# sony/aki

Measured on AMD Instinct MI355X. Metric: image+text tokens/sec forward, AKI-4B, 336px img + 512 txt, higher is better.
Workload: dtype bf16

## Files before the change

aki_amd/_lib.py:

```python
from __future__ import annotations

import ctypes as C
import os
from typing import Optional

_HERE = os.path.dirname(os.path.abspath(__file__))
LIB_PATH = os.environ.get("AKI_MI355X_LIB") or os.path.join(_HERE, "lib", "libaki_mi355x.so")
LAB_LIB_PATH = os.path.join(_HERE, "lib", "libaki_mi355x_lab.so")

AKI_DT_BF16, AKI_DT_F32, AKI_DT_FP8_E4M3, AKI_DT_W8A16, AKI_DT_W4A16 = 0, 1, 2, 3, 4
AKI_ACT_NONE, AKI_ACT_GELU_ERF, AKI_ACT_GELU_TANH, AKI_ACT_SWIGLU = 0, 1, 2, 3
AKI_DEAD_ROWS_ZERO, AKI_DEAD_ROWS_UNIFORM = 0, 1
AKI_MAX_RECTS = 8
AKI_PLAN_STRIDE = 12
AKI_ABI_VERSION = 17
AKI_LOGITS_PROCESS_MAX_V = 131072


class AkiError(RuntimeError):
    pass


class MmaRect(C.Structure):
    _fields_ = [("row_lo", C.c_int32), ("row_hi", C.c_int32), ("col_lo", C.c_int32), ("col_hi", C.c_int32)]
# ... 108 lines not shown
                ("cache_len", C.c_void_p), ("col_valid_bits", C.c_void_p), ("workspace", C.c_void_p), ("workspace_bytes", C.c_size_t),
                ("n_layers", C.c_int32), ("nwords", C.c_int32), ("d", C.c_int32), ("H", C.c_int32), ("Dh", C.c_int32), ("F", C.c_int32),
                ("capacity", C.c_int32), ("max_keys", C.c_int32), ("scale", C.c_float), ("rms_eps", C.c_float), ("dtype", C.c_int32),
                ("batch", C.c_int32)]


SIGNATURES = {
    "aki_strerror": (C.c_char_p, [C.c_int]),
    "aki_abi_version": (C.c_int, []),
    "aki_mma_attn_core_workspace_bytes": (C.c_size_t, [C.c_int32] * 5),
    "aki_mma_attn_core_fwd": (C.c_int, [C.POINTER(MmaAttnCoreArgs), C.c_void_p, C.c_size_t, C.c_void_p]),
    "aki_mma_attn_workspace_bytes": (C.c_size_t, [C.c_int32] * 5),
    "aki_mma_attn_fwd": (C.c_int, [C.POINTER(MmaAttnArgs), C.c_void_p, C.c_size_t, C.c_void_p]),
    "aki_qkv_rope_fwd": (C.c_int, [C.POINTER(MmaAttnArgs), C.c_void_p, C.c_void_p, C.c_void_p, C.c_void_p, C.c_size_t, C.c_void_p]),
    "aki_attn_fwd": (C.c_int, [C.POINTER(AttnArgs), C.c_void_p, C.c_size_t, C.c_void_p]),
    "aki_linear_fwd": (C.c_int, [C.POINTER(LinearArgs), C.c_void_p]),
    "aki_linear_stats_workspace_bytes": (C.c_size_t, [C.c_int32, C.c_int32]),
    "aki_linear_splitk_workspace_bytes": (C.c_size_t, [C.c_int32, C.c_int32, C.c_int32]),
    "aki_linear_stats_counter_bytes": (C.c_size_t, [C.c_int32]),
    "aki_row_stats": (C.c_int, [C.c_void_p, C.c_int32, C.c_int32, C.c_int32, C.c_float, C.c_void_p, C.c_void_p, C.c_int32, C.c_void_p]),
    "aki_rmsnorm_fwd": (C.c_int, [C.c_void_p, C.c_void_p, C.c_void_p, C.c_int32, C.c_int32, C.c_int32, C.c_int32,
                                  C.c_float, C.c_int32, C.c_void_p]),
    "aki_layernorm_fwd": (C.c_int, [C.c_void_p, C.c_void_p, C.c_void_p, C.c_void_p, C.c_int32, C.c_int32, C.c_int32,
                                    C.c_int32, C.c_float, C.c_int32, C.c_void_p]),
    "aki_patch_embed_workspace_bytes": (C.c_size_t, [C.c_int32] * 4),
    "aki_patch_embed_fwd": (C.c_int, [C.c_void_p] * 5 + [C.c_int32] * 6 + [C.c_void_p, C.c_size_t, C.c_void_p]),
    "aki_connector_mlp_workspace_bytes": (C.c_size_t, [C.c_int32] * 4),
    "aki_connector_mlp_fwd": (C.c_int, [C.c_void_p] * 6 + [C.c_int32] * 3 + [C.c_float, C.c_int32, C.c_void_p, C.c_size_t,
                                                                            C.c_void_p]),
    "aki_connector_proj_fwd": (C.c_int, [C.c_void_p] * 6 + [C.c_int32] * 3 + [C.c_float, C.c_int32, C.c_void_p, C.c_size_t,
# ... 40 lines not shown
    "aki_quant_rows_fp8": (C.c_int, [C.c_void_p, C.c_void_p, C.c_float, C.c_void_p, C.c_void_p] + [C.c_int32] * 4 + [C.c_void_p]),
    "aki_quant_mxfp4": (C.c_int, [C.c_void_p, C.c_int32, C.c_int32, C.c_int32, C.c_void_p, C.c_void_p, C.c_void_p]),
    "aki_linear_w4_fwd": (C.c_int, [C.POINTER(LinearArgs), C.c_void_p, C.c_void_p, C.c_float, C.c_void_p]),
    "aki_splice_plan": (C.c_int, [C.c_void_p, C.c_int32, C.c_int32, C.c_int64, C.c_int64, C.c_int32, C.c_void_p, C.c_void_p]),
    "aki_splice_fwd": (C.c_int, [C.POINTER(SpliceArgs), C.c_void_p]),
    "aki_mma_mask_dense": (C.c_int, [C.c_void_p, C.c_int32, C.c_void_p, C.c_void_p, C.c_int32, C.c_int32, C.c_void_p,
                                     C.c_void_p]),
    "aki_greedy_pick": (C.c_int, [C.c_void_p, C.c_int32, C.c_int32, C.c_int64, C.c_void_p, C.c_int32, C.c_int64, C.c_void_p, C.c_void_p, C.c_void_p, C.c_int32,
                                  C.c_void_p, C.c_void_p, C.c_int32, C.c_void_p, C.c_void_p]),
    "aki_decoder_stack_workspace_bytes": (C.c_size_t, [C.c_int32] * 7),
    "aki_decoder_stack_fwd": (C.c_int, [C.POINTER(DecoderStackArgs), C.c_void_p]),
    "aki_siglip_stack_workspace_bytes": (C.c_size_t, [C.c_int32] * 4),
    "aki_siglip_stack_fwd": (C.c_int, [C.POINTER(SiglipStackArgs), C.c_void_p]),
    "aki_perceiver_stack_workspace_bytes": (C.c_size_t, [C.c_int32] * 6),
    "aki_perceiver_stack_fwd": (C.c_int, [C.POINTER(PerceiverStackArgs), C.c_void_p]),
    "aki_greedy_pick_embed": (C.c_int, [C.c_void_p, C.c_int32, C.c_int32, C.c_int64, C.c_void_p, C.c_int32, C.c_int64, C.c_void_p, C.c_void_p, C.c_void_p, C.c_int32,
                                        C.c_void_p, C.c_void_p, C.c_int32, C.c_void_p, C.c_void_p, C.c_void_p, C.c_int64, C.c_int64, C.c_int32, C.c_void_p,
                                        C.c_void_p]),
    "aki_logits_process": (C.c_int, [C.c_void_p, C.c_int32, C.c_int32, C.c_int32, C.c_int64, C.c_void_p, C.c_int64, C.c_void_p, C.c_int32,
                                     C.c_void_p, C.c_void_p, C.c_int32, C.c_void_p, C.c_float, C.c_int32, C.c_int32, C.c_void_p, C.c_int32,
                                     C.c_void_p, C.c_int32, C.c_void_p, C.c_int32, C.c_void_p, C.c_void_p, C.c_int32, C.c_int32, C.c_void_p]),
    "aki_greedy_pick_processed": (C.c_int, [C.c_void_p, C.c_int32, C.c_int32, C.c_int64, C.c_void_p, C.c_int32, C.c_int64, C.c_void_p, C.c_void_p,
                                            C.c_void_p, C.c_int32, C.c_void_p, C.c_void_p, C.c_int32, C.c_void_p, C.c_void_p, C.c_void_p, C.c_int64,
                                            C.c_int64, C.c_int32, C.c_void_p, C.c_void_p, C.c_int64, C.c_float, C.c_int32, C.c_int32, C.c_void_p,
                                            C.c_int32, C.c_void_p, C.c_int32, C.c_void_p, C.c_void_p, C.c_int32, C.c_int32, C.c_void_p]),
    "aki_sample_pick": (C.c_int, [C.c_void_p, C.c_int32, C.c_int32, C.c_int64, C.c_void_p, C.c_int32, C.c_int64, C.c_void_p, C.c_void_p,
                                  C.c_void_p, C.c_int32, C.c_void_p, C.c_void_p, C.c_int32, C.c_void_p, C.c_void_p, C.c_void_p, C.c_int64,
                                  C.c_int64, C.c_int32, C.c_void_p, C.c_void_p, C.c_int64, C.c_float, C.c_int32, C.c_int32, C.c_void_p,
                                  C.c_int32, C.c_void_p, C.c_int32, C.c_void_p, C.c_void_p, C.c_int32, C.c_int32, C.c_int32, C.c_float,
                                  C.c_int32, C.c_float, C.c_uint64, C.c_uint64, C.c_void_p, C.c_int64, C.c_void_p]),
# ... 144 lines not shown
```

aki_amd/csrc/api.hip:

```cpp
#include "aki_device.h"

namespace aki {
int linear_bf16(const aki_linear_args* a, hipStream_t stream);
size_t linear_stats_ws_bytes(int M, int n_out);
size_t linear_stats_cnt_bytes(int M);
int row_stats_launch(const void* x, int rows, int cols, int ldx, float eps, float* rstd, float* mean, hipStream_t s);
int linear_f32(const aki_linear_args* a, hipStream_t stream);
int qkv_rope_bf16(const aki_mma_attn_args* a, void* q, void* k, void* v, hipStream_t stream);
int qkv_rope_fp8(const aki_mma_attn_args* a, void* q, void* k, void* v, hipStream_t stream);
int linear_fp8(const aki_linear_args* a, hipStream_t stream);
int quant_rows_fp8_launch(const void* x, const void* rms_w, float eps, void* q, float* scale, int rows, int cols, int ldx, int ldq,
                          hipStream_t s);
int qkv_rope_f32(const aki_mma_attn_args* a, void* q, void* k, void* v, float* tmp, hipStream_t stream);
int attn_core_bf16(const aki_mma_attn_core_args* a, void* ws, size_t ws_bytes, hipStream_t stream);
int attn_core_f32(const aki_mma_attn_core_args* a, void* ws, size_t ws_bytes, hipStream_t stream, int causal);
int attn_nc_bf16(const aki_attn_args* a, hipStream_t stream);
int gemv_bf16(const aki_linear_args* a, const void* rms_w, float eps, hipStream_t stream);
int skinny_gemm_bf16(const aki_linear_args* a, const void* rms_w, float eps, hipStream_t stream);
int skinny_gemm_w8(const aki_linear_args* a, const void* rms_w, float eps, hipStream_t stream);
int quant_mxfp4_launch(const void* w, int N, int K, int ldw, uint8_t* wq, uint8_t* ws, hipStream_t s);
int gemv_w4(const aki_linear_args* a, const uint8_t* ws, const void* rms_w, float eps, hipStream_t stream);
int skinny_gemm_w4(const aki_linear_args* a, const uint8_t* ws, const void* rms_w, float eps, hipStream_t stream);
size_t decode_attn_ws_bytes(int B, int H, int Dh, int cap);
int decode_attn_split_launch(const void* q_or_qkv, const float* cos, const float* sin, const int* len, void* kc, void* vc, void* o,
                             const uint64_t* vbits, int nwords, int B, int H, int cap, int max_keys, float scale, bool fused,
                             void* ws, size_t ws_bytes, hipStream_t s);
int rope_append_launch(const void* qkv, const float* cos, const float* sin, const int* pos, const int* cache_len, void* q_out,
                       void* k_cache, void* v_cache, int B, int H, int Dh, int cap, int dtype, hipStream_t s);
int kv_cache_quant_fp8_launch(const void* src, int src_cap, void* dst, float* scale, int dst_cap, int slabs, int rows, hipStream_t s);
int decode_attn_split_fp8kv_launch(const void* qkv, const float* cos, const float* sin, const int* len, void* kc, void* vc, float* ks, float* vs,
                                   void* o, const uint64_t* vbits, int nwords, int B, int H, int cap, int max_keys, float scale, void* ws,
// ... 148 lines not shown
int aki_attn_fwd(const aki_attn_args* a, void* ws, size_t ws_bytes, void* stream) {
  AKI_CLEAR_ERR();
  AKI_CHECK_ARG(a && a->q && a->k && a->v && a->o);
  AKI_CHECK_ARG(a->B > 0 && a->H > 0 && a->Lq > 0 && a->Lk > 0 && a->Dh > 0 && a->scale > 0.f && dtype_ok(a->dtype));
  if (a->dtype == AKI_DT_BF16) return attn_nc_bf16(a, (hipStream_t)stream);
  const int64_t Dh = a->Dh;
  if (a->q_stride_t != Dh || a->k_stride_t != Dh || a->v_stride_t != Dh || a->q_stride_h != (int64_t)a->Lq * Dh ||
      a->k_stride_h != (int64_t)a->Lk * Dh || a->v_stride_h != (int64_t)a->Lk * Dh || a->Lq != a->Lk)
    return AKI_ERR_UNSUPPORTED;
  aki_mma_attn_core_args c = {};
  c.q = a->q; c.k = a->k; c.v = a->v; c.o = a->o; c.B = a->B; c.H = a->H; c.L = a->Lq; c.Dh = a->Dh; c.scale = a->scale;
  c.dtype = AKI_DT_F32; c.dead_rows = AKI_DEAD_ROWS_ZERO;
  return attn_core_f32(&c, ws, ws_bytes, (hipStream_t)stream, 0);
}

static size_t qkv_bytes(int B, int H, int L, int Dh, int dtype) {
  return aki_align_up((size_t)B * H * L * Dh * aki_elt_size(dtype), 256);
}

size_t aki_mma_attn_workspace_bytes(int32_t B, int32_t H, int32_t L, int32_t Dh, int32_t dtype) {
  size_t n = 3 * qkv_bytes(B, H, L, Dh, dtype) + aki_mma_attn_core_workspace_bytes(B, H, L, Dh, dtype);
  if (dtype == AKI_DT_F32) n += 3 * qkv_bytes(B, H, L, Dh, dtype);
  return n;
}

static int check_fused(const aki_mma_attn_args* a) {
  AKI_CHECK_ARG(a && a->x && a->w_qkv && a->cos && a->sin);
  AKI_CHECK_ARG(a->B > 0 && a->H > 0 && a->L > 0 && a->Dh > 0 && a->d_model > 0);
  AKI_CHECK_ARG(a->ldx >= a->d_model && a->ldw >= a->d_model && a->pos_rows > 0);
  AKI_CHECK_ARG(a->position_ids || a->pos_rows >= a->L);
// ... 643 lines not shown
```

aki_amd/csrc/attn_nc_bf16.hip:

```cpp
#include "aki_device.h"

namespace aki {

struct AttnNcParams {
  const bf16_t* q;
  const bf16_t* k;
  const bf16_t* v;
  bf16_t* o;
  long q_sb, q_sh, q_st;
  long k_sb, k_sh, k_st;
  long v_sb, v_sh, v_st;
  int B, H, Lq, Lk;
  int nqt;
  float scale_log2;
  float* lse;
};

__device__ __forceinline__ float max3_nc(float a, float b, float c) {
  float r;
  asm("v_max3_f32 %0, %1, %2, %3" : "=v"(r) : "v"(a), "v"(b), "v"(c));
  return r;
}

template <int NW, int DH>
__global__ __launch_bounds__(NW * 64, 2) void attn_nc_bf16_kernel(const AttnNcParams p) {
  constexpr int BQ = NW * 32, NT = NW * 64;
  constexpr int KS = (DH + 15) / 16;
  constexpr int DT = (DH + 31) / 32;
  constexpr int CPR = DH / 8;
  constexpr int KROW = DH == 96 ? 208 : (DH == 72 ? 176 : (DH == 64 ? 144 : 80));
  constexpr int VROW = 192;
  constexpr int KTILE = 64 * KROW, VTILE = 64 * VROW;
  constexpr int NCHUNK = 64 * CPR;
  constexpr int NCH = (NCHUNK + NT - 1) / NT;
  __shared__ __attribute__((aligned(16))) char smem[2 * KTILE + 2 * VTILE];
  char* const sK = smem;
  char* const sV = smem + 2 * KTILE;

  const int tid = threadIdx.x, lane = tid & 63;
// ... 9 lines not shown
    const u32x4 z = {0u, 0u, 0u, 0u};
    if (KS * 16 > DH)
      for (int r = tid; r < 2 * 64; r += NT) *(u32x4*)(sK + (r >> 6) * KTILE + (r & 63) * KROW + CPR * 16) = z;
    if (DT * 32 > DH) {
      constexpr int PADC = 12 - CPR;
      for (int e = tid; e < 2 * 64 * PADC; e += NT) {
        const int buf = e / (64 * PADC), rr = (e / PADC) & 63, pc = e % PADC;
        *(u32x4*)(sV + buf * VTILE + rr * VROW + (CPR + pc) * 16) = z;
      }
    }
  }

  const bf16_t* qrow = p.q + (size_t)b * p.q_sb + (size_t)head * p.q_sh + (size_t)min(row, Lq - 1) * p.q_st;
  const char* kb = (const char*)(p.k + (size_t)b * p.k_sb + (size_t)head * p.k_sh);
  const char* vb = (const char*)(p.v + (size_t)b * p.v_sb + (size_t)head * p.v_sh);

  bf16x8 qf[KS];
#pragma unroll
  for (int ks = 0; ks < KS; ++ks) {
    const int d = min(16 * ks + 8 * h, DH - 8);
    qf[ks] = *(const bf16x8*)(qrow + d);
  }

  f32x16 o[DT];
#pragma unroll
  for (int dt = 0; dt < DT; ++dt)
#pragma unroll
    for (int r = 0; r < 16; ++r) o[dt][r] = 0.f;
  float m_run = -1e30f, l_part = 0.f;

  constexpr int KCP = KROW / 16, VCP = VROW / 16;
  constexpr int KN = (64 * KCP + NT - 1) / NT, VN = (64 * VCP + NT - 1) / NT;
  auto issue_tile = [&](int j, int buf) {
    const int c0 = j * 64;
#pragma unroll
    for (int i = 0; i < KN; ++i) {
      const int c = i * NT + tid;
      const int kr = c / KCP, kc = c - kr * KCP;
      if (kc < CPR && c < 64 * KCP) {
        const size_t trow = (size_t)min(c0 + kr, Lk - 1);
        __builtin_amdgcn_global_load_lds(AKI_GLOBAL_PTR(kb + trow * p.k_st * 2 + kc * 16), AKI_LDS_PTR(sK + buf * KTILE + (i * NT + wave * 64) * 16), 16, 0, 0);
      }
    }
#pragma unroll
    for (int i = 0; i < VN; ++i) {
      const int c = i * NT + tid;
      const int kr = c / VCP, kc = c - kr * VCP;
      if (kc < CPR && c < 64 * VCP) {
        const size_t trow = (size_t)min(c0 + kr, Lk - 1);
        __builtin_amdgcn_global_load_lds(AKI_GLOBAL_PTR(vb + trow * p.v_st * 2 + kc * 16), AKI_LDS_PTR(sV + buf * VTILE + (i * NT + wave * 64) * 16), 16, 0, 0);
      }
    }
  };

  const int koff = l31 * KROW + h * 16;
  const int voff = (4 * h + ((lane & 15) >> 2)) * VROW + (16 * ((lane >> 4) & 1) + 4 * (lane & 3)) * 2;
  const int jend = (Lk + 63) >> 6;

  __syncthreads();
  issue_tile(0, 0);
  __builtin_amdgcn_s_waitcnt(0x0F70);
  __syncthreads();

  for (int j = 0; j < jend; ++j) {
    if (j + 1 < jend) issue_tile(j + 1, (j + 1) & 1);
// ... 98 lines not shown
    bf16_t* orow = p.o + ((size_t)(b * Lq + row) * p.H + head) * DH + 4 * h;
#pragma unroll
    for (int dt = 0; dt < DT; ++dt)
#pragma unroll
      for (int q4 = 0; q4 < 4; ++q4) {
        const int d = dt * 32 + q4 * 8 + 4 * h;
        if (d < DH) {
          u32x2 pk = {pack_bf16x2(o[dt][4 * q4] * inv, o[dt][4 * q4 + 1] * inv), pack_bf16x2(o[dt][4 * q4 + 2] * inv, o[dt][4 * q4 + 3] * inv)};
          *(u32x2*)(orow + dt * 32 + q4 * 8) = pk;
        }
      }
    if (p.lse && h == 0) p.lse[(size_t)bh * Lq + row] = (m_run + __builtin_amdgcn_logf(l_tot)) * 0.69314718055994530942f;
  }
}

int attn_nc_bf16(const aki_attn_args* a, hipStream_t stream) {
  AttnNcParams p = {(const bf16_t*)a->q, (const bf16_t*)a->k, (const bf16_t*)a->v, (bf16_t*)a->o,
                    a->q_stride_b, a->q_stride_h, a->q_stride_t, a->k_stride_b, a->k_stride_h, a->k_stride_t,
                    a->v_stride_b, a->v_stride_h, a->v_stride_t, a->B, a->H, a->Lq, a->Lk, 0,
                    a->scale * 1.44269504088896340736f, a->lse};
  constexpr int NW = 4;
  p.nqt = (a->Lq + NW * 32 - 1) / (NW * 32);
  const long ss[] = {a->q_stride_b, a->q_stride_h, a->q_stride_t, a->k_stride_b, a->k_stride_h, a->k_stride_t,
                     a->v_stride_b, a->v_stride_h, a->v_stride_t};
  for (long s : ss)
    if (s % 8) return AKI_ERR_ALIGNMENT;
  AKI_CHECK_ALIGN16(a->q); AKI_CHECK_ALIGN16(a->k); AKI_CHECK_ALIGN16(a->v);
  if ((uintptr_t)a->o & 7) return AKI_ERR_ALIGNMENT;
  const dim3 grid(a->B * a->H * p.nqt), block(NW * 64);
  AKI_CLEAR_ERR();
  switch (a->Dh) {
    case 96: hipLaunchKernelGGL((attn_nc_bf16_kernel<NW, 96>), grid, block, 0, stream, p); break;
    case 72: hipLaunchKernelGGL((attn_nc_bf16_kernel<NW, 72>), grid, block, 0, stream, p); break;
    case 64: hipLaunchKernelGGL((attn_nc_bf16_kernel<NW, 64>), grid, block, 0, stream, p); break;
    case 32: hipLaunchKernelGGL((attn_nc_bf16_kernel<NW, 32>), grid, block, 0, stream, p); break;
    default: return AKI_ERR_UNSUPPORTED;
  }
  AKI_LAUNCH_CHECK();
  return AKI_OK;
}

}
```

aki_amd/csrc/stack.hip:

```cpp
#include <hip/hip_runtime.h>

#include "aki_device.h"

namespace {

inline char* carve(char*& p, size_t bytes) {
  char* r = p;
  p += aki_align_up(bytes, 256);
  return r;
}

}

extern "C" {

size_t aki_decoder_stack_workspace_bytes(int32_t B, int32_t H, int32_t L, int32_t Dh, int32_t d, int32_t F, int32_t keep_kv) {
  if (B <= 0 || H <= 0 || L <= 0 || Dh <= 0 || d <= 0 || F <= 0) return 0;
  const size_t M = (size_t)B * L, head = aki_align_up(M * H * Dh * 2, 256);
  return head * (keep_kv ? 1 : 3)
         + aki_align_up(M * (size_t)H * Dh * 2, 256)
         + 2 * aki_align_up(M * (size_t)d * 2, 256)
         + aki_align_up(M * (size_t)F * 2, 256)
         + 3 * aki_align_up(M * 4, 256)
         + aki_mma_attn_core_workspace_bytes(B, H, L, Dh, AKI_DT_BF16);
// ... 205 lines not shown
    rc = aki_attn_fwd(&at, attn_ws, attn_ws_bytes, stream);
    if (rc) return rc;
    aki_linear_args oa = {};
    oa.x = ao; oa.w = ly.w_out; oa.residual = cur; oa.y = lat[0]; oa.M = n2; oa.N = D; oa.K = inner; oa.ldx = inner; oa.ldw = inner; oa.ldy = D; oa.ldr = D;
    oa.act = AKI_ACT_NONE; oa.dtype = AKI_DT_BF16;
    rc = aki_linear_fwd(&oa, stream);
    if (rc) return rc;
    rc = aki_connector_mlp_fwd(lat[0], ly.ff_ln_w, ly.ff_ln_b, ly.ff_w1, ly.ff_w2, lat[1], n2, D, a->d_ff, a->eps, AKI_DT_BF16, mlp_ws, mlp_ws_bytes, stream);
    if (rc) return rc;
    cur = lat[1];
  }
  if (a->proj_w) return aki_connector_proj_fwd(cur, a->norm_w, a->norm_b, a->proj_w, a->proj_b, a->out, n2, D, a->D_out, a->eps, AKI_DT_BF16, mlp_ws, mlp_ws_bytes, stream);
  return aki_layernorm_fwd(cur, a->norm_w, a->norm_b, a->out, n2, D, D, D, a->eps, AKI_DT_BF16, stream);
}

}
```

aki_amd/helpers.py:

```python
from __future__ import annotations

from dataclasses import dataclass
from typing import Optional

import torch
import torch.nn.functional as F
from torch import nn

from . import ops
from . import train_ops as TR

try:
    from transformers.modeling_outputs import CausalLMOutputWithPast
except Exception:
    @dataclass
    class CausalLMOutputWithPast:
        loss: Optional[torch.Tensor] = None
        logits: Optional[torch.Tensor] = None
        past_key_values: Optional[object] = None
        hidden_states: Optional[object] = None
        attentions: Optional[object] = None

        def __getitem__(self, i):
            return [v for v in (self.loss, self.logits, self.past_key_values) if v is not None][i]
# ... 82 lines not shown
            self.layers.append(nn.ModuleList([PerceiverAttention(dim=dim, dim_head=dim_head, heads=heads),
                                              FeedForward(dim=dim, mult=ff_mult)]))
        self.norm = nn.LayerNorm(dim)

    use_layer_stack = True

    def _can_stack(self, x) -> bool:
        if not (self.use_layer_stack and ops.stack_enabled() and x.is_cuda and x.dtype == torch.bfloat16 and x.is_contiguous()):
            return False
        eps = self.norm.eps
        for attn, ff in self.layers:
            if (attn.norm_media.eps != eps or attn.norm_latents.eps != eps or ff[0].eps != eps
                    or attn.heads != self.layers[0][0].heads or attn.dim_head != self.layers[0][0].dim_head):
                return False
        return not ops.python_must_run_between(self.layers)

    def _forward_stack(self, x, latents):
        tb = getattr(self, "_stack_table", None)
        if tb is None:
            tb = self._stack_table = ops.LayerTable(ops.L.PerceiverLayer)
        live = []
        for attn, ff in self.layers:
            live += [attn.norm_media.weight, attn.norm_media.bias, attn.norm_latents.weight, attn.norm_latents.bias, attn.to_q.weight,
                     attn.to_kv.weight, attn.to_out.weight, ff[0].weight, ff[0].bias, ff[1].weight, ff[3].weight]
        sig = (tuple(map(id, live)), ops.params_signature(live))
        if tb.sig != sig:
            rows = []
            for attn, ff in self.layers:
                rows.append((attn.norm_media.weight, attn.norm_media.bias, attn.norm_latents.weight, attn.norm_latents.bias, attn.to_q.weight,
                             attn.to_kv.weight, attn.to_out.weight, ff[0].weight, ff[0].bias, ff[1].weight, ff[3].weight))
            for r in rows:
                for t_ in r:
                    if t_ is not None and not t_.is_contiguous():
                        raise ops.AkiError("perceiver stack: weights must be contiguous")
            tb.get(rows)
            tb.sig = sig
        a0 = self.layers[0][0]
        proj = self.projection
        return ops.perceiver_stack(tb.arr, len(self.layers), x.reshape(-1, x.shape[-1]), latents.reshape(-1, latents.shape[-1]), self.norm.weight, self.norm.bias,
                                   None if proj is None else proj.weight, None if proj is None else proj.bias, a0.heads, a0.dim_head,
                                   self.layers[0][1][1].weight.shape[0], a0.scale, self.norm.eps)

    def forward(self, x):
        b, T, Fr, v = x.shape[:4]
        if exists(self.frame_embs):
            x = x + self.frame_embs[:Fr][None, None, :, None, :]
        x = x.reshape(b, T, Fr * v, x.shape[-1])
        if exists(self.media_time_embs):
            x = x + self.media_time_embs[:T]
        latents = self.latents.to(x.dtype)[None, None].expand(b, T, -1, -1).contiguous()
        if _ag(latents, *self.parameters()):
            for attn, ff in self.layers:
                latents = attn(x, latents)
                hmid = TR.GeluFn.apply(TR.linear(TR.layernorm(latents, ff[0].weight, ff[0].bias, ff[0].eps), ff[1].weight))
                latents = TR.linear(hmid, ff[3].weight, None, latents)
            latents = TR.layernorm(latents, self.norm.weight, self.norm.bias, self.norm.eps)
            if exists(self.projection):
                return TR.linear(latents, self.projection.weight, self.projection.bias, None)
            return latents
        if b * T == 1 and self._can_stack(x):
            return self._forward_stack(x, latents).view(b, T, latents.shape[2], -1)
        for attn, ff in self.layers:
            latents = attn(x, latents)
            latents = ops.connector_mlp(latents, ff[0].weight, ff[0].bias, ff[1].weight, ff[3].weight, ff[0].eps)
        if exists(self.projection):
            return ops.connector_proj(latents, self.norm.weight, self.norm.bias, self.projection.weight,
                                      self.projection.bias, self.norm.eps)
        return ops.layernorm(latents, self.norm.weight, self.norm.bias, self.norm.eps)


def _table_dims(given: Optional[torch.Tensor], declared_rows, declared_cols, what: str):
    if given is None:
        if declared_rows is None or declared_cols is None:
            raise AssertionError(f"{what}: without a ready-made tensor both sizes have to be given")
        return int(declared_rows), int(declared_cols)
    rows, cols = given.shape
    for declared, actual in ((declared_rows, rows), (declared_cols, cols)):
        if declared is not None and declared != actual:
            raise AssertionError(f"{what}: the tensor is {rows} x {cols}, which contradicts the declared size {declared}")
# ... 102 lines not shown
```

aki_amd/ops.py:

```python
from __future__ import annotations

import ctypes as C
import threading
from dataclasses import dataclass
from typing import Optional, Tuple

import torch

from . import _lib as L
from ._lib import AkiError

ACT_NONE, ACT_GELU_ERF, ACT_GELU_TANH, ACT_SWIGLU = L.AKI_ACT_NONE, L.AKI_ACT_GELU_ERF, L.AKI_ACT_GELU_TANH, L.AKI_ACT_SWIGLU
DEAD_ROWS_ZERO, DEAD_ROWS_UNIFORM = L.AKI_DEAD_ROWS_ZERO, L.AKI_DEAD_ROWS_UNIFORM


def _dt(t: torch.Tensor) -> int:
    if t.dtype == torch.bfloat16:
        return L.AKI_DT_BF16
    if t.dtype == torch.float32:
        return L.AKI_DT_F32
    raise AkiError(f"unsupported dtype {t.dtype}: the AKI HIP path computes in bf16 or f32")


def _dev(*ts: Optional[torch.Tensor]) -> torch.device:
# ... 254 lines not shown
    q, k, v = q.contiguous(), k.contiguous(), v.contiguous()
    o = torch.empty((B, Lq, H * Dh), dtype=q.dtype, device=dev)
    lse = torch.empty((B, H, Lq), dtype=torch.float32, device=dev) if return_lse else None
    lib = L.load()
    ws = _ws(lib.aki_mma_attn_core_workspace_bytes(B, H, Lq, Dh, _dt(q)), dev)
    a = L.MmaAttnCoreArgs(_ptr(q), _ptr(k), _ptr(v), _ptr(o), _ptr(lse), _ptr(table.rects), _ptr(table.col_valid_bits),
                          _ptr(table.seq_lens), table.max_rects, B, H, Lq, Dh, float(scale), _dt(q), dead_rows,
                          0 if cap == Lq else cap)
    end = _TAP.begin(("mma_attn_core", B, H, Lq, Dh)) if (_TAP is not None and _TAP.want(("mma_attn_core",))) else None
    L.check(lib.aki_mma_attn_core_fwd(C.byref(a), _ptr(ws), ws.numel(), _stream()), "aki_mma_attn_core_fwd")
    if end is not None:
        end.record()
    return (o, lse) if return_lse else o


def attention(q: torch.Tensor, k: torch.Tensor, v: torch.Tensor, scale: float, return_lse: bool = False):
    dev = _dev(q, k, v)
    B, Lq, H, Dh = q.shape
    Lk = k.shape[1]
    o = torch.empty((B, Lq, H * Dh), dtype=q.dtype, device=dev)
    lib = L.load()
    if q.dtype == torch.float32:
        if Lq != Lk:
            qp = torch.zeros((B, Lk, H, Dh), dtype=q.dtype, device=dev)
            qp[:, :Lq] = q
            return attention(qp, k, v, scale)[:, :Lq].contiguous()
        q, k, v = (t_.permute(0, 2, 1, 3).contiguous() for t_ in (q, k, v))
        st = lambda t_: (t_.stride(0), t_.stride(1), t_.stride(2))
    else:
        for t_ in (q, k, v):
            if t_.stride(3) != 1:
                raise AkiError("attention: channel stride must be 1")
        st = lambda t_: (t_.stride(0), t_.stride(2), t_.stride(1))
    ws = _ws(B * H * Dh * 4 + 256, dev)
# ... 648 lines not shown
    if x.dtype != torch.bfloat16 or not x.is_contiguous() or not latents.is_contiguous() or x.dim() != 2 or latents.dim() != 2:
        raise AkiError("perceiver_stack: contiguous bf16 [n, D] tensors")
    lib = L.load()
    n1, D = x.shape
    n2 = latents.shape[0]
    D_out = D if proj_w is None else proj_w.shape[0]
    out = torch.empty((n2, D_out), dtype=x.dtype, device=dev)
    ws = _scratch(int(lib.aki_perceiver_stack_workspace_bytes(n1, n2, D, heads, dim_head, d_ff)), dev)
    off = (-ws.data_ptr()) % 256
    a = L.PerceiverStackArgs(table_arr, n_layers, _ptr(x), _ptr(latents), _ptr(norm_w), _ptr(norm_b), _ptr(proj_w), _ptr(proj_b), _ptr(out), n1, n2, D, heads,
                             dim_head, d_ff, D_out, float(scale), float(eps), ws.data_ptr() + off, ws.numel() - off)
    L.check(lib.aki_perceiver_stack_fwd(C.byref(a), _stream()), "aki_perceiver_stack_fwd")
    return out


def quant_rows_fp8(x: torch.Tensor, rms_weight: Optional[torch.Tensor] = None, eps: float = 0.0):
    dev = _dev(x, rms_weight)
    if x.dtype != torch.bfloat16:
        raise AkiError("quant_rows_fp8 takes bf16 input")
    x2 = _rows2d(x)
    rows, cols = x2.shape
    q = torch.empty((rows, cols), dtype=torch.uint8, device=dev)
    s = torch.empty((rows,), dtype=torch.float32, device=dev)
    L.check(L.load().aki_quant_rows_fp8(_ptr(x2), _ptr(rms_weight), float(eps), _ptr(q), _ptr(s), rows, cols, x2.stride(0),
                                        q.stride(0), _stream()), "aki_quant_rows_fp8")
    return q, s


def linear_fp8(xq: torch.Tensor, xs: torch.Tensor, wq: torch.Tensor, ws: torch.Tensor, bias: Optional[torch.Tensor] = None,
               residual: Optional[torch.Tensor] = None, act: int = ACT_NONE, out_shape=None) -> torch.Tensor:
# ... 307 lines not shown
```

include/aki_mi355x.h:

```cpp
#ifndef AKI_MI355X_H
#define AKI_MI355X_H

#include <stddef.h>
#include <stdint.h>

#ifdef __cplusplus
extern "C" {
#endif

#define AKI_ABI_VERSION 17

typedef enum {
  AKI_OK = 0,
  AKI_ERR_INVALID_ARG = -1,
  AKI_ERR_UNSUPPORTED = -2,
  AKI_ERR_ALIGNMENT = -3,
  AKI_ERR_WORKSPACE = -4,
  AKI_ERR_LAUNCH = -5
} aki_status;

typedef enum {
  AKI_DT_BF16 = 0,
  AKI_DT_F32 = 1,
  AKI_DT_FP8_E4M3 = 2,
// ... 73 lines not shown
typedef struct {
  const void* q;
  const void* k;
  const void* v;
  void* o;
  int64_t q_stride_b, q_stride_h, q_stride_t;
  int64_t k_stride_b, k_stride_h, k_stride_t;
  int64_t v_stride_b, v_stride_h, v_stride_t;
  int32_t B, H, Lq, Lk, Dh;
  float scale;
  int32_t dtype;
  float* lse;
} aki_attn_args;

int aki_attn_fwd(const aki_attn_args* args, void* workspace, size_t workspace_bytes, void* stream);

typedef struct {
  const void* x;
  const void* w;
  const void* bias;
  const void* residual;
  void* y;
  int32_t M, N, K;
  int32_t ldx, ldw, ldy, ldr;
  int32_t res_row_mod;
  int32_t act;
  int32_t dtype;
  const float* x_scale;
  const float* w_scale;
  const void* w2;
// ... 306 lines not shown
  const void* norm_w;
  const void* norm_b;
  const void* proj_w;
  const void* proj_b;
  void* out;
  int32_t n1, n2, D, heads, dim_head, d_ff, D_out;
  float scale;
  float eps;
  void* workspace;
  size_t workspace_bytes;
} aki_perceiver_stack_args;

size_t aki_perceiver_stack_workspace_bytes(int32_t n1, int32_t n2, int32_t D, int32_t heads, int32_t dim_head, int32_t d_ff);
int aki_perceiver_stack_fwd(const aki_perceiver_stack_args* args, void* stream);

int aki_greedy_pick_embed(const void* logits, int32_t B, int32_t V, int64_t ld, const int64_t* eos_ids, int32_t n_eos, int64_t pad_token_id,
                          uint8_t* done, int64_t* next_ids, int64_t* tokens, int32_t tokens_ld, int32_t* cache_len, const int32_t* start_len,
                          int32_t advance, int32_t* done_at, const void* embed_weight, const void* additional_weight, int64_t max_original_id,
                          int64_t num_additional, int32_t d, void* next_embeds, void* stream);

#define AKI_LOGITS_PROCESS_MAX_V 131072
int aki_logits_process(const void* logits, int32_t dtype, int32_t B, int32_t V, int64_t ld, float* out, int64_t ld_out, const int64_t* tokens,
                       int32_t tokens_ld, const int32_t* cache_len, const int32_t* start_len, int32_t step, const uint8_t* done,
                       float repetition_penalty, int32_t no_repeat_ngram_size, int32_t min_length, const int64_t* eos_ids, int32_t n_eos,
                       const int64_t* suppress_ids, int32_t n_suppress, const int64_t* begin_suppress_ids, int32_t n_begin_suppress,
                       const int64_t* bad_ids, const int32_t* bad_offsets, int32_t n_bad, int32_t n_bad_ids, void* stream);

int aki_greedy_pick_processed(const void* logits, int32_t B, int32_t V, int64_t ld, const int64_t* eos_ids, int32_t n_eos, int64_t pad_token_id,
                              uint8_t* done, int64_t* next_ids, int64_t* tokens, int32_t tokens_ld, int32_t* cache_len, const int32_t* start_len,
                              int32_t advance, int32_t* done_at, const void* embed_weight, const void* additional_weight, int64_t max_original_id,
// ... 19 lines not shown
```

Before: 131,000.

## Split perceiver attention into media and latent KV segments to avoid concat

Adds a two-segment key/value attention kernel so the perceiver resampler can attend over media keys and latent keys without materializing the concatenated KV tensor. The latent K/V projection is merged with the Q projection into one stacked GEMM per layer. Optionally, all layers' media KV projections can be folded into one GEMM with the layernorm applied as row scale and shift. The cost is a per-load branch in the kernel, cached stacked weight copies, and a path limited to head dim 64.

```diff
diff --git a/aki_amd/_lib.py b/aki_amd/_lib.py
--- a/aki_amd/_lib.py
+++ b/aki_amd/_lib.py
@@ -146,6 +146,7 @@
     "aki_mma_attn_fwd": (C.c_int, [C.POINTER(MmaAttnArgs), C.c_void_p, C.c_size_t, C.c_void_p]),
     "aki_qkv_rope_fwd": (C.c_int, [C.POINTER(MmaAttnArgs), C.c_void_p, C.c_void_p, C.c_void_p, C.c_void_p, C.c_size_t, C.c_void_p]),
     "aki_attn_fwd": (C.c_int, [C.POINTER(AttnArgs), C.c_void_p, C.c_size_t, C.c_void_p]),
+    "aki_attn_kv2_fwd": (C.c_int, [C.POINTER(AttnArgs), C.c_void_p, C.c_void_p] + [C.c_int64] * 6 + [C.c_int32, C.c_void_p]),
     "aki_linear_fwd": (C.c_int, [C.POINTER(LinearArgs), C.c_void_p]),
     "aki_linear_stats_workspace_bytes": (C.c_size_t, [C.c_int32, C.c_int32]),
     "aki_linear_splitk_workspace_bytes": (C.c_size_t, [C.c_int32, C.c_int32, C.c_int32]),
@@ -216,6 +217,8 @@
     "aki_siglip_stack_fwd": (C.c_int, [C.POINTER(SiglipStackArgs), C.c_void_p]),
     "aki_perceiver_stack_workspace_bytes": (C.c_size_t, [C.c_int32] * 6),
     "aki_perceiver_stack_fwd": (C.c_int, [C.POINTER(PerceiverStackArgs), C.c_void_p]),
+    "aki_perceiver_stack_shared_workspace_bytes": (C.c_size_t, [C.c_int32] * 7),
+    "aki_perceiver_stack_shared_fwd": (C.c_int, [C.POINTER(PerceiverStackArgs)] + [C.c_void_p] * 5),
     "aki_greedy_pick_embed": (C.c_int, [C.c_void_p, C.c_int32, C.c_int32, C.c_int64, C.c_void_p, C.c_int32, C.c_int64, C.c_void_p, C.c_void_p, C.c_void_p, C.c_int32,
                                         C.c_void_p, C.c_void_p, C.c_int32, C.c_void_p, C.c_void_p, C.c_void_p, C.c_int64, C.c_int64, C.c_int32, C.c_void_p,
                                         C.c_void_p]),
diff --git a/aki_amd/csrc/api.hip b/aki_amd/csrc/api.hip
--- a/aki_amd/csrc/api.hip
+++ b/aki_amd/csrc/api.hip
@@ -15,6 +15,7 @@
 int attn_core_bf16(const aki_mma_attn_core_args* a, void* ws, size_t ws_bytes, hipStream_t stream);
 int attn_core_f32(const aki_mma_attn_core_args* a, void* ws, size_t ws_bytes, hipStream_t stream, int causal);
 int attn_nc_bf16(const aki_attn_args* a, hipStream_t stream);
+int attn_nc_bf16_kv2(const aki_attn_args* a, const void* k2, const void* v2, const int64_t* s2, int Lk1, hipStream_t stream);
 int gemv_bf16(const aki_linear_args* a, const void* rms_w, float eps, hipStream_t stream);
 int skinny_gemm_bf16(const aki_linear_args* a, const void* rms_w, float eps, hipStream_t stream);
 int skinny_gemm_w8(const aki_linear_args* a, const void* rms_w, float eps, hipStream_t stream);
@@ -193,6 +194,16 @@
   return attn_core_f32(&c, ws, ws_bytes, (hipStream_t)stream, 0);
 }
 
+int aki_attn_kv2_fwd(const aki_attn_args* a, const void* k2, const void* v2, int64_t k2_stride_b, int64_t k2_stride_h, int64_t k2_stride_t,
+                     int64_t v2_stride_b, int64_t v2_stride_h, int64_t v2_stride_t, int32_t Lk1, void* stream) {
+  AKI_CLEAR_ERR();
+  AKI_CHECK_ARG(a && a->q && a->k && a->v && a->o && k2 && v2);
+  AKI_CHECK_ARG(a->B > 0 && a->H > 0 && a->Lq > 0 && a->Dh > 0 && a->scale > 0.f && Lk1 > 0 && Lk1 < a->Lk);
+  if (a->dtype != AKI_DT_BF16) return AKI_ERR_UNSUPPORTED;
+  const int64_t s2[6] = {k2_stride_b, k2_stride_h, k2_stride_t, v2_stride_b, v2_stride_h, v2_stride_t};
+  return attn_nc_bf16_kv2(a, k2, v2, s2, Lk1, (hipStream_t)stream);
+}
+
 static size_t qkv_bytes(int B, int H, int L, int Dh, int dtype) {
   return aki_align_up((size_t)B * H * L * Dh * aki_elt_size(dtype), 256);
 }
diff --git a/aki_amd/csrc/attn_nc_bf16.hip b/aki_amd/csrc/attn_nc_bf16.hip
--- a/aki_amd/csrc/attn_nc_bf16.hip
+++ b/aki_amd/csrc/attn_nc_bf16.hip
@@ -14,6 +14,11 @@
   int nqt;
   float scale_log2;
   float* lse;
+  const bf16_t* k2;
+  const bf16_t* v2;
+  long k2_sb, k2_sh, k2_st;
+  long v2_sb, v2_sh, v2_st;
+  int Lk1;
 };
 
 __device__ __forceinline__ float max3_nc(float a, float b, float c) {
@@ -22,7 +27,7 @@
   return r;
 }
 
-template <int NW, int DH>
+template <int NW, int DH, bool SEG2 = false>
 __global__ __launch_bounds__(NW * 64, 2) void attn_nc_bf16_kernel(const AttnNcParams p) {
   constexpr int BQ = NW * 32, NT = NW * 64;
   constexpr int KS = (DH + 15) / 16;
@@ -62,6 +67,8 @@
   const bf16_t* qrow = p.q + (size_t)b * p.q_sb + (size_t)head * p.q_sh + (size_t)min(row, Lq - 1) * p.q_st;
   const char* kb = (const char*)(p.k + (size_t)b * p.k_sb + (size_t)head * p.k_sh);
   const char* vb = (const char*)(p.v + (size_t)b * p.v_sb + (size_t)head * p.v_sh);
+  const char* kb2 = SEG2 ? (const char*)(p.k2 + (size_t)b * p.k2_sb + (size_t)head * p.k2_sh) : nullptr;
+  const char* vb2 = SEG2 ? (const char*)(p.v2 + (size_t)b * p.v2_sb + (size_t)head * p.v2_sh) : nullptr;
 
   bf16x8 qf[KS];
 #pragma unroll
@@ -86,8 +93,10 @@
       const int c = i * NT + tid;
       const int kr = c / KCP, kc = c - kr * KCP;
       if (kc < CPR && c < 64 * KCP) {
-        const size_t trow = (size_t)min(c0 + kr, Lk - 1);
-        __builtin_amdgcn_global_load_lds(AKI_GLOBAL_PTR(kb + trow * p.k_st * 2 + kc * 16), AKI_LDS_PTR(sK + buf * KTILE + (i * NT + wave * 64) * 16), 16, 0, 0);
+        const int trow = min(c0 + kr, Lk - 1);
+        const char* src = kb + (size_t)trow * p.k_st * 2;
+        if (SEG2 && trow >= p.Lk1) src = kb2 + (size_t)(trow - p.Lk1) * p.k2_st * 2;
+        __builtin_amdgcn_global_load_lds(AKI_GLOBAL_PTR(src + kc * 16), AKI_LDS_PTR(sK + buf * KTILE + (i * NT + wave * 64) * 16), 16, 0, 0);
       }
     }
 #pragma unroll
@@ -95,8 +104,10 @@
       const int c = i * NT + tid;
       const int kr = c / VCP, kc = c - kr * VCP;
       if (kc < CPR && c < 64 * VCP) {
-        const size_t trow = (size_t)min(c0 + kr, Lk - 1);
-        __builtin_amdgcn_global_load_lds(AKI_GLOBAL_PTR(vb + trow * p.v_st * 2 + kc * 16), AKI_LDS_PTR(sV + buf * VTILE + (i * NT + wave * 64) * 16), 16, 0, 0);
+        const int trow = min(c0 + kr, Lk - 1);
+        const char* src = vb + (size_t)trow * p.v_st * 2;
+        if (SEG2 && trow >= p.Lk1) src = vb2 + (size_t)(trow - p.Lk1) * p.v2_st * 2;
+        __builtin_amdgcn_global_load_lds(AKI_GLOBAL_PTR(src + kc * 16), AKI_LDS_PTR(sV + buf * VTILE + (i * NT + wave * 64) * 16), 16, 0, 0);
       }
     }
   };
@@ -225,7 +236,7 @@
   }
 }
 
-int attn_nc_bf16(const aki_attn_args* a, hipStream_t stream) {
+static int attn_nc_launch(const aki_attn_args* a, const void* k2, const void* v2, const int64_t* s2, int Lk1, hipStream_t stream) {
   AttnNcParams p = {(const bf16_t*)a->q, (const bf16_t*)a->k, (const bf16_t*)a->v, (bf16_t*)a->o,
                     a->q_stride_b, a->q_stride_h, a->q_stride_t, a->k_stride_b, a->k_stride_h, a->k_stride_t,
                     a->v_stride_b, a->v_stride_h, a->v_stride_t, a->B, a->H, a->Lq, a->Lk, 0,
@@ -239,6 +250,19 @@
   AKI_CHECK_ALIGN16(a->q); AKI_CHECK_ALIGN16(a->k); AKI_CHECK_ALIGN16(a->v);
   if ((uintptr_t)a->o & 7) return AKI_ERR_ALIGNMENT;
   const dim3 grid(a->B * a->H * p.nqt), block(NW * 64);
+  if (k2) {
+    if (a->Dh != 64) return AKI_ERR_UNSUPPORTED;
+    for (int i = 0; i < 6; ++i)
+      if (s2[i] % 8) return AKI_ERR_ALIGNMENT;
+    AKI_CHECK_ALIGN16(k2); AKI_CHECK_ALIGN16(v2);
+    p.k2 = (const bf16_t*)k2; p.v2 = (const bf16_t*)v2;
+    p.k2_sb = s2[0]; p.k2_sh = s2[1]; p.k2_st = s2[2]; p.v2_sb = s2[3]; p.v2_sh = s2[4]; p.v2_st = s2[5];
+    p.Lk1 = Lk1;
+    AKI_CLEAR_ERR();
+    hipLaunchKernelGGL((attn_nc_bf16_kernel<NW, 64, true>), grid, block, 0, stream, p);
+    AKI_LAUNCH_CHECK();
+    return AKI_OK;
+  }
   AKI_CLEAR_ERR();
   switch (a->Dh) {
     case 96: hipLaunchKernelGGL((attn_nc_bf16_kernel<NW, 96>), grid, block, 0, stream, p); break;
@@ -251,4 +275,10 @@
   return AKI_OK;
 }
 
-}
+int attn_nc_bf16(const aki_attn_args* a, hipStream_t stream) { return attn_nc_launch(a, nullptr, nullptr, nullptr, 0, stream); }
+
+int attn_nc_bf16_kv2(const aki_attn_args* a, const void* k2, const void* v2, const int64_t* s2, int Lk1, hipStream_t stream) {
+  return attn_nc_launch(a, k2, v2, s2, Lk1, stream);
+}
+
+}
diff --git a/aki_amd/csrc/stack.hip b/aki_amd/csrc/stack.hip
--- a/aki_amd/csrc/stack.hip
+++ b/aki_amd/csrc/stack.hip
@@ -243,4 +243,90 @@
   return aki_layernorm_fwd(cur, a->norm_w, a->norm_b, a->out, n2, D, D, D, a->eps, AKI_DT_BF16, stream);
 }
 
-}
+size_t aki_perceiver_stack_shared_workspace_bytes(int32_t n1, int32_t n2, int32_t D, int32_t heads, int32_t dim_head, int32_t d_ff, int32_t n_layers) {
+  if (n1 <= 0 || n2 <= 0 || D <= 0 || heads <= 0 || dim_head <= 0 || d_ff <= 0 || n_layers <= 0) return 0;
+  const size_t inner = (size_t)heads * dim_head;
+  return 2 * aki_align_up((size_t)n1 * 4, 256) + aki_align_up((size_t)n1 * n_layers * 2 * inner * 2, 256) + aki_align_up((size_t)n1 * D * 2, 256) +
+         aki_align_up((size_t)n2 * D * 2, 256) +
+         aki_align_up((size_t)n2 * 3 * inner * 2, 256) + aki_align_up((size_t)n2 * inner * 2, 256) + 2 * aki_align_up((size_t)n2 * D * 2, 256) +
+         aki_connector_mlp_workspace_bytes(n2, D, d_ff, AKI_DT_BF16);
+}
+
+int aki_perceiver_stack_shared_fwd(const aki_perceiver_stack_args* a, const void* w_kv_media, const void* b_kv_media, const float* c_kv_media,
+                                   const void* w_qkv_latents, void* stream) {
+  AKI_CLEAR_ERR();
+  AKI_CHECK_ARG(a && a->layers && a->n_layers > 0 && a->x && a->latents && a->out && a->norm_w && a->workspace);
+  const bool fold = w_kv_media != nullptr;
+  AKI_CHECK_ARG(w_qkv_latents && (!fold || (b_kv_media && c_kv_media)));
+  AKI_CHECK_ARG(a->n1 > 0 && a->n2 > 0 && a->D > 0 && a->heads > 0 && a->dim_head > 0 && a->d_ff > 0 && a->eps > 0.f && a->scale > 0.f);
+  AKI_CHECK_ARG(!a->proj_w || a->D_out > 0);
+  for (int i = 0; i < a->n_layers; ++i) {
+    const aki_perceiver_layer& ly = a->layers[i];
+    AKI_CHECK_ARG(ly.norm_latents_w && ly.w_out && ly.ff_ln_w && ly.ff_w1 && ly.ff_w2 && (fold || (ly.norm_media_w && ly.w_kv)));
+  }
+  if (a->workspace_bytes < aki_perceiver_stack_shared_workspace_bytes(a->n1, a->n2, a->D, a->heads, a->dim_head, a->d_ff, a->n_layers) ||
+      ((uintptr_t)a->workspace & 255))
+    return AKI_ERR_WORKSPACE;
+  const int n1 = a->n1, n2 = a->n2, D = a->D, inner = a->heads * a->dim_head, nl = a->n_layers, ldkv = (fold ? nl : 1) * 2 * inner;
+  char* w = (char*)a->workspace;
+  float* rstd = (float*)carve(w, (size_t)n1 * 4);
+  float* mean = (float*)carve(w, (size_t)n1 * 4);
+  char* kvm = carve(w, (size_t)n1 * nl * 2 * inner * 2);
+  void* xn = carve(w, (size_t)n1 * D * 2);
+  void* ln = carve(w, (size_t)n2 * D * 2);
+  char* qkv = carve(w, (size_t)n2 * 3 * inner * 2);
+  void* ao = carve(w, (size_t)n2 * inner * 2);
+  void* lat[2] = {carve(w, (size_t)n2 * D * 2), carve(w, (size_t)n2 * D * 2)};
+  void* mlp_ws = w;
+  const size_t mlp_ws_bytes = aki_connector_mlp_workspace_bytes(n2, D, a->d_ff, AKI_DT_BF16);
+  int rc;
+  if (fold) {
+    rc = aki_row_stats(a->x, n1, D, D, a->eps, rstd, mean, AKI_DT_BF16, stream);
+    if (rc) return rc;
+    aki_linear_args ma = {};
+    ma.x = a->x; ma.w = w_kv_media; ma.bias = b_kv_media; ma.y = kvm; ma.M = n1; ma.N = ldkv; ma.K = D; ma.ldx = D; ma.ldw = D; ma.ldy = ldkv;
+    ma.act = AKI_ACT_NONE; ma.dtype = AKI_DT_BF16; ma.row_scale = rstd; ma.row_shift = mean; ma.col_shift = c_kv_media;
+    rc = aki_linear_fwd(&ma, stream);
+    if (rc) return rc;
+  }
+  const void* cur = a->latents;
+  for (int i = 0; i < nl; ++i) {
+    const aki_perceiver_layer& ly = a->layers[i];
+    const char* kl = fold ? kvm + (size_t)i * 2 * inner * 2 : kvm;
+    if (!fold) {
+      rc = aki_layernorm_fwd(a->x, ly.norm_media_w, ly.norm_media_b, xn, n1, D, D, D, a->eps, AKI_DT_BF16, stream);
+      if (rc) return rc;
+      aki_linear_args ma = {};
+      ma.x = xn; ma.w = ly.w_kv; ma.y = kvm; ma.M = n1; ma.N = 2 * inner; ma.K = D; ma.ldx = D; ma.ldw = D; ma.ldy = ldkv; ma.act = AKI_ACT_NONE; ma.dtype = AKI_DT_BF16;
+      rc = aki_linear_fwd(&ma, stream);
+      if (rc) return rc;
+    }
+    rc = aki_layernorm_fwd(cur, ly.norm_latents_w, ly.norm_latents_b, ln, n2, D, D, D, a->eps, AKI_DT_BF16, stream);
+    if (rc) return rc;
+    aki_linear_args qa = {};
+    qa.x = ln; qa.w = (const char*)w_qkv_latents + (size_t)i * 3 * inner * D * 2; qa.y = qkv; qa.M = n2; qa.N = 3 * inner; qa.K = D; qa.ldx = D; qa.ldw = D;
+    qa.ldy = 3 * inner; qa.act = AKI_ACT_NONE; qa.dtype = AKI_DT_BF16;
+    rc = aki_linear_fwd(&qa, stream);
+    if (rc) return rc;
+    aki_attn_args at = {};
+    at.q = qkv; at.k = kl; at.v = kl + (size_t)inner * 2; at.o = ao;
+    at.q_stride_b = (int64_t)n2 * 3 * inner; at.q_stride_h = a->dim_head; at.q_stride_t = 3 * inner;
+    at.k_stride_b = at.v_stride_b = (int64_t)n1 * ldkv; at.k_stride_h = at.v_stride_h = a->dim_head; at.k_stride_t = at.v_stride_t = ldkv;
+    at.B = 1; at.H = a->heads; at.Lq = n2; at.Lk = n1 + n2; at.Dh = a->dim_head; at.scale = a->scale; at.dtype = AKI_DT_BF16;
+    rc = aki_attn_kv2_fwd(&at, qkv + (size_t)inner * 2, qkv + (size_t)2 * inner * 2, at.q_stride_b, a->dim_head, 3 * inner, at.q_stride_b, a->dim_head,
+                          3 * inner, n1, stream);
+    if (rc) return rc;
+    aki_linear_args oa = {};
+    oa.x = ao; oa.w = ly.w_out; oa.residual = cur; oa.y = lat[0]; oa.M = n2; oa.N = D; oa.K = inner; oa.ldx = inner; oa.ldw = inner; oa.ldy = D; oa.ldr = D;
+    oa.act = AKI_ACT_NONE; oa.dtype = AKI_DT_BF16;
+    rc = aki_linear_fwd(&oa, stream);
+    if (rc) return rc;
+    rc = aki_connector_mlp_fwd(lat[0], ly.ff_ln_w, ly.ff_ln_b, ly.ff_w1, ly.ff_w2, lat[1], n2, D, a->d_ff, a->eps, AKI_DT_BF16, mlp_ws, mlp_ws_bytes, stream);
+    if (rc) return rc;
+    cur = lat[1];
+  }
+  if (a->proj_w) return aki_connector_proj_fwd(cur, a->norm_w, a->norm_b, a->proj_w, a->proj_b, a->out, n2, D, a->D_out, a->eps, AKI_DT_BF16, mlp_ws, mlp_ws_bytes, stream);
+  return aki_layernorm_fwd(cur, a->norm_w, a->norm_b, a->out, n2, D, D, D, a->eps, AKI_DT_BF16, stream);
+}
+
+}
diff --git a/aki_amd/helpers.py b/aki_amd/helpers.py
--- a/aki_amd/helpers.py
+++ b/aki_amd/helpers.py
@@ -120,6 +120,64 @@
                     or attn.heads != self.layers[0][0].heads or attn.dim_head != self.layers[0][0].dim_head):
                 return False
         return not ops.python_must_run_between(self.layers)
+
+    share_media_kv = True
+    fold_media_norm = False
+
+    def _can_share(self, x) -> bool:
+        if not (self.share_media_kv and x.is_cuda and x.dtype == torch.bfloat16 and len(self.layers) > 0):
+            return False
+        a0 = self.layers[0][0]
+        if a0.dim_head != 64:
+            return False
+        for attn, _ in self.layers:
+            if (attn.norm_media.eps != a0.norm_media.eps or attn.heads != a0.heads or attn.dim_head != a0.dim_head
+                    or attn.norm_media.bias is None or attn.to_kv.weight.dtype != torch.bfloat16):
+                return False
+        return not ops.python_must_run_between(self.layers)
+
+    def _shared_weights(self):
+        from .siglip import _epoch, fold_layernorm
+        live = []
+        for attn, _ in self.layers:
+            live += [attn.norm_media.weight, attn.norm_media.bias, attn.to_q.weight, attn.to_kv.weight]
+        fold = bool(self.fold_media_norm)
+        sig = (fold, _epoch(live), tuple(map(id, live)), ops.params_signature(live))
+        hit = getattr(self, "_shared_cache", None)
+        if hit is None or hit[0] != sig:
+            with torch.no_grad():
+                w_all = b_all = c_all = None
+                if fold:
+                    folded = [fold_layernorm(attn.to_kv.weight.detach(), None, attn.norm_media) for attn, _ in self.layers]
+                    w_all = torch.cat([f[0] for f in folded], 0).contiguous()
+                    b_all = torch.cat([f[1] for f in folded], 0).contiguous()
+                    c_all = torch.cat([f[2][: f[0].shape[0]] for f in folded], 0).contiguous()
+                w_qkv = torch.stack([torch.cat((attn.to_q.weight.detach(), attn.to_kv.weight.detach()), 0) for attn, _ in self.layers], 0).contiguous()
+            hit = self._shared_cache = (sig, (w_all, b_all, c_all, w_qkv))
+        return hit[1]
+
+    def _forward_shared(self, x, latents):
+        b, T, n1, D = x.shape
+        n2 = latents.shape[2]
+        a0 = self.layers[0][0]
+        h, dh, nl = a0.heads, a0.dim_head, len(self.layers)
+        w_all, b_all, c_all, w_qkv = self._shared_weights()
+        if w_all is not None:
+            st = ops.row_stats(x, a0.norm_media.eps, ln=True)
+            kvm = ops.linear(x, w_all, bias=b_all, row_scale=st.rstd, row_shift=st.mean, col_shift=c_all).view(b * T, n1, nl, 2, h, dh)
+        for i, (attn, ff) in enumerate(self.layers):
+            if w_all is not None:
+                km, vm = kvm[:, :, i, 0], kvm[:, :, i, 1]
+            else:
+                xn = ops.layernorm(x, attn.norm_media.weight, attn.norm_media.bias, attn.norm_media.eps)
+                kv = ops.linear(xn, attn.to_kv.weight).view(b * T, n1, 2, h, dh)
+                km, vm = kv[:, :, 0], kv[:, :, 1]
+            ln = ops.layernorm(latents, attn.norm_latents.weight, attn.norm_latents.bias, attn.norm_latents.eps)
+            qkv = ops.linear(ln, w_qkv[i]).view(b * T, n2, 3, h, dh)
+            out = ops.attention(qkv[:, :, 0], km, vm, attn.scale, k2=qkv[:, :, 1], v2=qkv[:, :, 2])
+            latents = ops.linear(out.view(b, T, n2, h * dh), attn.to_out.weight, residual=latents)
+            latents = ops.connector_mlp(latents, ff[0].weight, ff[0].bias, ff[1].weight, ff[3].weight, ff[0].eps)
+        return latents
 
     def _forward_stack(self, x, latents):
         tb = getattr(self, "_stack_table", None)
@@ -143,6 +201,10 @@
             tb.sig = sig
         a0 = self.layers[0][0]
         proj = self.projection
+        if self._can_share(x):
+            return ops.perceiver_stack_shared(tb.arr, len(self.layers), x.reshape(-1, x.shape[-1]), latents.reshape(-1, latents.shape[-1]), self.norm.weight,
+                                              self.norm.bias, None if proj is None else proj.weight, None if proj is None else proj.bias, a0.heads,
+                                              a0.dim_head, self.layers[0][1][1].weight.shape[0], a0.scale, self.norm.eps, *self._shared_weights())
         return ops.perceiver_stack(tb.arr, len(self.layers), x.reshape(-1, x.shape[-1]), latents.reshape(-1, latents.shape[-1]), self.norm.weight, self.norm.bias,
                                    None if proj is None else proj.weight, None if proj is None else proj.bias, a0.heads, a0.dim_head,
                                    self.layers[0][1][1].weight.shape[0], a0.scale, self.norm.eps)
@@ -166,9 +228,12 @@
             return latents
         if b * T == 1 and self._can_stack(x):
             return self._forward_stack(x, latents).view(b, T, latents.shape[2], -1)
-        for attn, ff in self.layers:
-            latents = attn(x, latents)
-            latents = ops.connector_mlp(latents, ff[0].weight, ff[0].bias, ff[1].weight, ff[3].weight, ff[0].eps)
+        if self._can_share(x):
+            latents = self._forward_shared(x, latents)
+        else:
+            for attn, ff in self.layers:
+                latents = attn(x, latents)
+                latents = ops.connector_mlp(latents, ff[0].weight, ff[0].bias, ff[1].weight, ff[3].weight, ff[0].eps)
         if exists(self.projection):
             return ops.connector_proj(latents, self.norm.weight, self.norm.bias, self.projection.weight,
                                       self.projection.bias, self.norm.eps)
diff --git a/aki_amd/ops.py b/aki_amd/ops.py
--- a/aki_amd/ops.py
+++ b/aki_amd/ops.py
@@ -292,10 +292,28 @@
     return (o, lse) if return_lse else o
 
 
-def attention(q: torch.Tensor, k: torch.Tensor, v: torch.Tensor, scale: float, return_lse: bool = False):
-    dev = _dev(q, k, v)
+def attention(q: torch.Tensor, k: torch.Tensor, v: torch.Tensor, scale: float, return_lse: bool = False,
+              k2: Optional[torch.Tensor] = None, v2: Optional[torch.Tensor] = None):
+    dev = _dev(q, k, v, k2, v2)
     B, Lq, H, Dh = q.shape
     Lk = k.shape[1]
+    if (k2 is None) != (v2 is None):
+        raise AkiError("attention: k2 and v2 come together")
+    if k2 is not None:
+        if q.dtype != torch.bfloat16 or k2.shape != v2.shape or k2.shape[0] != B or k2.shape[2:] != k.shape[2:] or v.shape != k.shape:
+            raise AkiError("attention: the second key / value segment is bf16 [B, Lk2, H, Dh]")
+        for t_ in (q, k, v, k2, v2):
+            if t_.stride(3) != 1:
+                raise AkiError("attention: channel stride must be 1")
+        st = lambda t_: (t_.stride(0), t_.stride(2), t_.stride(1))
+        o = torch.empty((B, Lq, H * Dh), dtype=q.dtype, device=dev)
+        lse = torch.empty((B, H, Lq), dtype=torch.float32, device=dev) if return_lse else None
+        a = L.AttnArgs(_ptr(q), _ptr(k), _ptr(v), _ptr(o), *st(q), *st(k), *st(v), B, H, Lq, Lk + k2.shape[1], Dh, float(scale), _dt(q), _ptr(lse))
+        end = _TAP.begin(("attention", B, H, Lq, Lk + k2.shape[1], Dh)) if (_TAP is not None and _TAP.want(("attention",))) else None
+        L.check(L.load().aki_attn_kv2_fwd(C.byref(a), _ptr(k2), _ptr(v2), *st(k2), *st(v2), Lk, _stream()), "aki_attn_kv2_fwd")
+        if end is not None:
+            end.record()
+        return (o, lse) if return_lse else o
     o = torch.empty((B, Lq, H * Dh), dtype=q.dtype, device=dev)
     lib = L.load()
     if q.dtype == torch.float32:
@@ -974,6 +992,33 @@
     return out
 
 
+def perceiver_stack_shared(table_arr, n_layers: int, x: torch.Tensor, latents: torch.Tensor, norm_w, norm_b, proj_w, proj_b, heads: int, dim_head: int,
+                           d_ff: int, scale: float, eps: float, w_kv_media: Optional[torch.Tensor], b_kv_media: Optional[torch.Tensor],
+                           c_kv_media: Optional[torch.Tensor], w_qkv_latents: torch.Tensor) -> torch.Tensor:
+    dev = _dev(x, latents, norm_w, norm_b, proj_w, proj_b, w_kv_media, b_kv_media, c_kv_media, w_qkv_latents)
+    if x.dtype != torch.bfloat16 or not x.is_contiguous() or not latents.is_contiguous() or x.dim() != 2 or latents.dim() != 2:
+        raise AkiError("perceiver_stack_shared: contiguous bf16 [n, D] tensors")
+    lib = L.load()
+    n1, D = x.shape
+    n2 = latents.shape[0]
+    inner = heads * dim_head
+    if tuple(w_qkv_latents.shape) != (n_layers, 3 * inner, D) or not w_qkv_latents.is_contiguous():
+        raise AkiError("perceiver_stack_shared: stacked weights of the wrong shape")
+    if w_kv_media is not None and (
+            tuple(w_kv_media.shape) != (n_layers * 2 * inner, D) or b_kv_media.numel() != n_layers * 2 * inner or c_kv_media.numel() < n_layers * 2 * inner
+            or c_kv_media.dtype != torch.float32 or not (w_kv_media.is_contiguous() and b_kv_media.is_contiguous() and c_kv_media.is_contiguous())):
+        raise AkiError("perceiver_stack_shared: stacked weights of the wrong shape")
+    D_out = D if proj_w is None else proj_w.shape[0]
+    out = torch.empty((n2, D_out), dtype=x.dtype, device=dev)
+    ws = _scratch(int(lib.aki_perceiver_stack_shared_workspace_bytes(n1, n2, D, heads, dim_head, d_ff, n_layers)), dev)
+    off = (-ws.data_ptr()) % 256
+    a = L.PerceiverStackArgs(table_arr, n_layers, _ptr(x), _ptr(latents), _ptr(norm_w), _ptr(norm_b), _ptr(proj_w), _ptr(proj_b), _ptr(out), n1, n2, D, heads,
+                             dim_head, d_ff, D_out, float(scale), float(eps), ws.data_ptr() + off, ws.numel() - off)
+    L.check(lib.aki_perceiver_stack_shared_fwd(C.byref(a), _ptr(w_kv_media), _ptr(b_kv_media), _ptr(c_kv_media), _ptr(w_qkv_latents), _stream()),
+            "aki_perceiver_stack_shared_fwd")
+    return out
+
+
 def quant_rows_fp8(x: torch.Tensor, rms_weight: Optional[torch.Tensor] = None, eps: float = 0.0):
     dev = _dev(x, rms_weight)
     if x.dtype != torch.bfloat16:
diff --git a/include/aki_mi355x.h b/include/aki_mi355x.h
--- a/include/aki_mi355x.h
+++ b/include/aki_mi355x.h
@@ -111,6 +111,9 @@
 } aki_attn_args;
 
 int aki_attn_fwd(const aki_attn_args* args, void* workspace, size_t workspace_bytes, void* stream);
+
+int aki_attn_kv2_fwd(const aki_attn_args* args, const void* k2, const void* v2, int64_t k2_stride_b, int64_t k2_stride_h, int64_t k2_stride_t,
+                     int64_t v2_stride_b, int64_t v2_stride_h, int64_t v2_stride_t, int32_t Lk1, void* stream);
 
 typedef struct {
   const void* x;
@@ -447,6 +450,10 @@
 size_t aki_perceiver_stack_workspace_bytes(int32_t n1, int32_t n2, int32_t D, int32_t heads, int32_t dim_head, int32_t d_ff);
 int aki_perceiver_stack_fwd(const aki_perceiver_stack_args* args, void* stream);
 
+size_t aki_perceiver_stack_shared_workspace_bytes(int32_t n1, int32_t n2, int32_t D, int32_t heads, int32_t dim_head, int32_t d_ff, int32_t n_layers);
+int aki_perceiver_stack_shared_fwd(const aki_perceiver_stack_args* args, const void* w_kv_media, const void* b_kv_media, const float* c_kv_media,
+                                   const void* w_qkv_latents, void* stream);
+
 int aki_greedy_pick_embed(const void* logits, int32_t B, int32_t V, int64_t ld, const int64_t* eos_ids, int32_t n_eos, int64_t pad_token_id,
                           uint8_t* done, int64_t* next_ids, int64_t* tokens, int32_t tokens_ld, int32_t* cache_len, const int32_t* start_len,
                           int32_t advance, int32_t* done_at, const void* embed_weight, const void* additional_weight, int64_t max_original_id,
```

Result: no change. 131,300 (median of 6 runs) (+0.2%).
